# mfkiwl/coxgraph

Hardware: AMD Instinct MI355X
Metric: 640x480 depth frames/sec fused (TSDF, 5 cm voxels) per node; submap registrations/sec reported alongside (higher is better)
Workload: dtype f32; 1 GPU; configs[1]: 1 client per GPU, 640x480 synthetic depth stream, 5 cm voxels, merged integrator semantics (the reference's configured method is fast; bit-exact vs CPU oracle), points resident in HBM; points_per_frame=307200, method=merged, clients=1

## Files before the change

### coxgraph_amd/capi.py

```python
import ctypes as C
import os
import numpy as np

COX_OK = 0
STATUS = {
    0: "COX_OK", -1: "COX_ERR_INVALID_ARG", -2: "COX_ERR_NO_DEVICE", -3: "COX_ERR_OUT_OF_MEMORY",
    -4: "COX_ERR_POOL_EXHAUSTED", -5: "COX_ERR_INDEX_RANGE", -6: "COX_ERR_UNSUPPORTED",
    -7: "COX_ERR_BUFFER_TOO_SMALL", -8: "COX_ERR_INTERNAL", -9: "COX_ERR_COMM",
}
METHODS = {"simple": 0, "merged": 1, "fast": 2, "projective": 3}
QUERY_MODES = {"nearest": 0, "interpolate": 1, "adaptive": 2}
Q_VALUE, Q_TRILINEAR, Q_GRADIENT = 1, 2, 4
R_HIT, R_NORMAL, R_COLOR, R_BUDGET = 1, 2, 4, 8
VOXELS_PER_BLOCK = 4096


class CoxError(RuntimeError):
    def __init__(self, status, what):
        super().__init__(f"{what}: {STATUS.get(status, status)}")
        self.status = status


class TsdfConfig(C.Structure):
    _fields_ = [
# ... 49 lines not shown


def _ptr(t):
    if t is None:
        return None
    return C.c_void_p(t.data_ptr() if hasattr(t, "data_ptr") else int(t))


def _stream(s):
    return C.c_void_p(getattr(s, "cuda_stream", s) or 0)


def _pose(T):
    T = np.ascontiguousarray(T, np.float32)
    assert T.shape == (7,)
    return T


def _intrinsics(w, h, K):
    if K is None:
        from . import synth
        K = synth.INTRINSICS[(w, h)]
    K = np.ascontiguousarray(K, np.float32)
    assert K.shape == (4,)
    return K


def _config(eng, Struct, default_symbol, overrides):
    c = Struct()
    eng.fn(default_symbol, None)(C.byref(c))
    for k, v in overrides.items():
        if not hasattr(c, k):
            raise AttributeError(k)
        if isinstance(getattr(c, k), C.Array):
            v = type(getattr(c, k))(*np.asarray(v).ravel().tolist())
        setattr(c, k, v)
    return c


def _esdf_config(eng, max_distance_m=None, min_distance_m=None, default_distance_m=None, min_weight=None):
    if max_distance_m is not None and default_distance_m is None:
        default_distance_m = max_distance_m
    given = dict(max_distance_m=max_distance_m, min_distance_m=min_distance_m, default_distance_m=default_distance_m, min_weight=min_weight)
    return _config(eng, EsdfConfig, "esdf_config_default", {k: v for k, v in given.items() if v is not None})


class Engine:

    def __init__(self, lib_path, prefix):
        if not os.path.exists(lib_path):
            raise FileNotFoundError(lib_path)
        self.lib = C.CDLL(lib_path)
        self.prefix = prefix
        self.path = lib_path
        self._status_fns = {}

    def fn(self, name, restype=C.c_int):
        f = getattr(self.lib, self.prefix + name)
        f.restype = restype
        return f

    def has(self, name):
        return hasattr(self.lib, self.prefix + name)

    def check(self, status, what):
        if status != COX_OK:
            raise CoxError(status, what)

    def call(self, name, *args):
        try:
            f = self._status_fns[name]
        except KeyError:
            f = self._status_fns[name] = self.lib[self.prefix + name]
            f.restype = C.c_int
        status = f(*args)
        if status != COX_OK:
            raise CoxError(status, name)

    def default_config(self, **overrides):
        return _config(self, TsdfConfig, "tsdf_config_default", overrides)

    def device_count(self):
        return int(self.fn("device_count")()) if self.has("device_count") else 0


class _Handle:
    _destroy = None
    _hattr = "h"
    _borrows = ()
    eng = None
    h = None

    @classmethod
    def _adopt(cls, eng, handle, **attrs):
        self = cls.__new__(cls)
        self.eng = eng
        setattr(self, cls._hattr, handle)
        for k, v in attrs.items():
            setattr(self, k, v)
        return self

    def _guard(self, name):
        for a in self._borrows:
            if not getattr(self, a).h:
                raise CoxError(-1, name + " (the layer is closed)")
        return getattr(self, self._hattr)

    def _call(self, name, *args):
        self.eng.call(name, self._guard(name), *args)

    def _download(self, name, shapes, place=lambda arrays, cap: (*arrays, cap), query=None, also_ok=()):
        h, f, n = self._guard(name), self.eng.fn(name), C.c_uint64()
        status = f(h, *place([None] * len(shapes), C.c_uint64(0)), C.byref(n))
        if status not in also_ok:
            self.eng.check(status, query or name)
        out = tuple(np.zeros((int(n.value), *shape), dtype) for shape, dtype in shapes)
        if n.value:
            self.eng.check(f(h, *place([_fp(a) for a in out], C.c_uint64(n.value)), C.byref(n)), name)
        return out

    def close(self):
        h = getattr(self, self._hattr)
        if h:
            self.eng.fn(self._destroy, None)(h)
            setattr(self, self._hattr, C.c_void_p())

    def __del__(self):
        try:
            self.close()
        except Exception:
            pass


class Layer(_Handle):
    _destroy = "layer_destroy"

    def __init__(self, eng, voxel_size, voxels_per_side=16, device=0, capacity_blocks=0):
        self.eng = eng
        self.voxel_size = float(voxel_size)
        self.h = C.c_void_p()
        eng.call("layer_create", C.c_float(voxel_size), C.c_int(voxels_per_side), C.c_int(device), C.c_uint64(capacity_blocks), C.byref(self.h))

    def clear(self):
        self._call("layer_clear")

    def stats(self):
        n, b = C.c_uint64(), C.c_uint64()
        self._call("layer_stats", C.byref(n), C.byref(b))
        return int(n.value), int(b.value)

    def download(self):
        return self._download("layer_download", (((3,), np.int32), ((VOXELS_PER_BLOCK, 3), np.uint32)), query="layer_download(query)")

    def merge_from(self, other, T_B_A=None):
        self.eng.call("layer_merge", other.h, None if T_B_A is None else _fp(_pose(T_B_A)), self.h)

    def registration_points(self, min_voxel_weight=1.0, max_voxel_distance=0.3):
        return self._download("layer_registration_points", (((5,), np.float32),),
                              lambda a, cap: (C.c_float(min_voxel_weight), C.c_float(max_voxel_distance), *a, cap))[0]

    def surface_obb(self):
        mn, mx, n = np.zeros(3, np.float32), np.zeros(3, np.float32), C.c_uint64()
        self._call("layer_surface_obb", _fp(mn), _fp(mx), C.byref(n))
        return mn, mx, int(n.value)

    def esdf(self, max_distance_m=None, min_distance_m=None, default_distance_m=None, min_weight=None):
# ... 1342 lines not shown
```

### coxgraph_amd/csrc/cox_frontend.hpp

```cpp
#pragma once

constexpr u32 kDepthTile = 2048;
__device__ __forceinline__ bool depth_valid(float d) { return isfinite(d) && d > 0.0f; }
__global__ void __launch_bounds__(256) k_depth_count(const float* __restrict__ depth, u32 n, u32* __restrict__ tile_sums) {
  __shared__ u32 lds[4];
  const u32 n_tiles = (n + kDepthTile - 1) / kDepthTile;
  for (u32 tile = blockIdx.x; tile < n_tiles; tile += gridDim.x) {
    u32 c = 0;
#pragma unroll
    for (u32 q = 0; q < kDepthTile / 256; ++q) {
      const u32 i = tile * kDepthTile + q * 256 + threadIdx.x;
      c += (i < n && depth_valid(depth[i])) ? 1u : 0u;
    }
    u32 tot;
    (void)block_exclusive_scan<4>(c, &tot, lds);
    if (threadIdx.x == 0) tile_sums[tile] = tot;
  }
}
__global__ void __launch_bounds__(256) k_depth_points(const float* __restrict__ depth, const uint8_t* __restrict__ rgba, int w, int h, float fx, float fy,
                                                      float cx, float cy, const u32* __restrict__ tile_sums, float* __restrict__ xyz,
                                                      uint8_t* __restrict__ rgba_out, u32* __restrict__ n_out) {
  __shared__ u32 lds[4], lds2[4];
  const u32 n = static_cast<u32>(w) * static_cast<u32>(h);
  const u32 n_tiles = (n + kDepthTile - 1) / kDepthTile;
  for (u32 tile = blockIdx.x; tile < n_tiles; tile += gridDim.x) {
    u32 below = 0;
    for (u32 t = threadIdx.x; t < tile; t += 256) below += tile_sums[t];
    u32 base;
    (void)block_exclusive_scan<4>(below, &base, lds2);
    const u32 i0 = tile * kDepthTile + threadIdx.x * 8;
    float d[8];
    u32 c = 0;
#pragma unroll
    for (u32 q = 0; q < 8; ++q) {
      d[q] = (i0 + q < n) ? depth[i0 + q] : 0.0f;
      c += depth_valid(d[q]) ? 1u : 0u;
    }
    u32 tot;
    u32 o = base + block_exclusive_scan<4>(c, &tot, lds);
#pragma unroll
    for (u32 q = 0; q < 8; ++q) {
      if (!depth_valid(d[q])) continue;
      const u32 i = i0 + q;
      const u32 u = i % static_cast<u32>(w), v = i / static_cast<u32>(w);
      const float xn = (static_cast<float>(u) - cx) / fx;
      const float yn = (static_cast<float>(v) - cy) / fy;
      xyz[3 * o] = d[q] * xn;
      xyz[3 * o + 1] = d[q] * yn;
      xyz[3 * o + 2] = d[q];
      if (rgba_out) reinterpret_cast<u32*>(rgba_out)[o] = rgba ? reinterpret_cast<const u32*>(rgba)[i] : 0u;
      ++o;
    }
    if (tile + 1 == n_tiles && threadIdx.x == 0) *n_out = base + tot;
  }
}

typedef u32 U32x4 __attribute__((ext_vector_type(4)));
constexpr int kCopyGroups = 8;
struct HostSegment {
  U32x4* dst;
  const U32x4* src;
  size_t n16;
  u32 tail_words;
};
__device__ __forceinline__ void copy_segment_from_host(const HostSegment& g) {
  const size_t stride = static_cast<size_t>(gridDim.x) * blockDim.x;
  size_t i = blockIdx.x * static_cast<size_t>(blockDim.x) + threadIdx.x;
  for (; i + 3 * stride < g.n16; i += 4 * stride) {
    const U32x4 a = __builtin_nontemporal_load(&g.src[i]);
    const U32x4 b = __builtin_nontemporal_load(&g.src[i + stride]);
    const U32x4 c = __builtin_nontemporal_load(&g.src[i + 2 * stride]);
    const U32x4 d = __builtin_nontemporal_load(&g.src[i + 3 * stride]);
    g.dst[i] = a;
    g.dst[i + stride] = b;
    g.dst[i + 2 * stride] = c;
    g.dst[i + 3 * stride] = d;
  }
  for (; i < g.n16; i += stride) g.dst[i] = __builtin_nontemporal_load(&g.src[i]);
  if (blockIdx.x == 0 && threadIdx.x < g.tail_words)
    reinterpret_cast<u32*>(g.dst + g.n16)[threadIdx.x] = reinterpret_cast<const u32*>(g.src + g.n16)[threadIdx.x];
}
__global__ void __launch_bounds__(256) k_copy_from_host(const HostSegment a, const HostSegment b) {
  copy_segment_from_host(a);
  if (b.dst) copy_segment_from_host(b);
}

__global__ void __launch_bounds__(256) k_selftest_division(u64 n, u64 seed, u32* __restrict__ mismatches) {
  u64 bad = 0;
  for (u64 i = blockIdx.x * static_cast<u64>(blockDim.x) + threadIdx.x; i < n; i += static_cast<u64>(gridDim.x) * blockDim.x) {
    u64 z = seed + 0x9E3779B97F4A7C15ull * (i + 1);
    z = (z ^ (z >> 30)) * 0xBF58476D1CE4E5B9ull;
    z = (z ^ (z >> 27)) * 0x94D049BB133111EBull;
    z ^= z >> 31;
    const u32 a = static_cast<u32>(z), b = static_cast<u32>(z >> 32);
    float D, N;
    if ((i & 3) == 0) {
      D = static_cast<float>((b % 200000u) + 1u);
    } else {
      D = __uint_as_float(((b & 0x007FFFFFu) | (((b >> 23) % 80u + 87u) << 23)));
    }
    N = __uint_as_float((a & 0x807FFFFFu) | ((((a >> 23) & 0xFFu) % 80u + 87u) << 23));
    const float r0 = __builtin_amdgcn_rcpf(D);
    const float r = __builtin_fmaf(__builtin_fmaf(-D, r0, 1.0f), r0, r0);
    const float q0 = N * r;
    const float e0 = __builtin_fmaf(-D, q0, N);
    const float q1 = __builtin_fmaf(e0, r, q0);
    const float e1 = __builtin_fmaf(-D, q1, N);
    const float q = __builtin_fmaf(e1, r, q1);
    const float ref = N / D;
    if (__float_as_uint(q) != __float_as_uint(ref)) ++bad;
  }
  if (bad) atomicAdd(mismatches, static_cast<u32>(bad > 0xFFFFFFFFull ? 0xFFFFFFFFull : bad));
}

__global__ void __launch_bounds__(1024) k_scan_small(const u32* __restrict__ in, u32* __restrict__ out, const u32* __restrict__ d_n, u32 n_max,
                                                     u32* __restrict__ d_total) {
  __shared__ u32 lds[16];
  const u32 n = min(*d_n, n_max);
  u32 carry = 0;
  for (u32 base = 0; base < n; base += 1024 * 4) {
    const u32 i0 = base + threadIdx.x * 4;
    u32 v[4], sum = 0;
#pragma unroll
    for (int q = 0; q < 4; ++q) {
      v[q] = (i0 + q < n) ? in[i0 + q] : 0u;
      sum += v[q];
    }
    u32 total;
    u32 ex = carry + block_exclusive_scan<16>(sum, &total, lds);
#pragma unroll
    for (int q = 0; q < 4; ++q) {
      if (i0 + q < n) out[i0 + q] = ex;
      ex += v[q];
    }
    carry += total;
  }
  if (threadIdx.x == 0) *d_total = carry;
}

__global__ void __launch_bounds__(1024) k_scan_small2(const u32* __restrict__ in_a, u32* __restrict__ out_a, u32* __restrict__ total_a, const u32* __restrict__ in_b,
                                                      u32* __restrict__ out_b, u32* __restrict__ total_b, const u32* __restrict__ d_n, u32 n_max) {
  __shared__ u32 lds[16];
  const u32 n = min(*d_n, n_max);
  for (int which = 0; which < 2; ++which) {
    const u32* __restrict__ in = which ? in_b : in_a;
    u32* __restrict__ out = which ? out_b : out_a;
    u32 carry = 0;
    for (u32 base = 0; base < n; base += 1024 * 4) {
      const u32 i0 = base + threadIdx.x * 4;
      u32 v[4], sum = 0;
#pragma unroll
      for (int q = 0; q < 4; ++q) {
        v[q] = (i0 + q < n) ? in[i0 + q] : 0u;
        sum += v[q];
      }
      u32 total;
      u32 ex = carry + block_exclusive_scan<16>(sum, &total, lds);
#pragma unroll
      for (int q = 0; q < 4; ++q) {
        if (i0 + q < n) out[i0 + q] = ex;
        ex += v[q];
      }
      carry += total;
    }
    if (threadIdx.x == 0) *(which ? total_b : total_a) = carry;
  }
}
```

### coxgraph_amd/csrc/cox_integrator.hip

```cpp
#include <hip/hip_runtime.h>

#include <algorithm>
#include <chrono>
#include <cmath>
#include <cstring>
#include <limits>
#include <new>
#include <string>
#include <vector>

#include "../../include/coxgraph_hip_history.h"
#include "../../include/coxgraph_hip_selftest.h"
#include "cox_host.hpp"
#include "cox_plan.hpp"
#include "cox_sort.hpp"
#include "cox_threads.hpp"

using namespace cox;
using cox_plan::IntegratorPlan;
using cox_plan::LayerUpdate;

#include "cox_frame.hpp"
#include "cox_raygen.hpp"
#include "cox_walk.hpp"
#include "cox_pieces.hpp"
#include "cox_fast.hpp"
#include "cox_apply_records.hpp"
#include "cox_apply_tile.hpp"
#include "cox_frontend.hpp"

static_assert(cox_plan::kAxisCapSmall == kAxisCapSmall && cox_plan::kTileShift == kTileShift && cox_plan::kBigChunk == kBigChunk &&
                  cox_plan::kBigChunkMin == kBigChunkMin && cox_plan::kFastMaxRounds == kFastMaxRounds && cox_plan::kFastShortMax == kFastShortMax &&
                  cox_plan::kFastRelaxGroups == kFastRelaxGroups && cox_plan::kCopyGroups == kCopyGroups,
              "cox_plan.hpp decides with the kernels' own constants");

constexpr int kStatRing = 8;
constexpr int kFrameSets = 6;
constexpr int kStageSets = 3;
constexpr int kInputSets = kFrameSets;
using cox_plan::kNumStages;

struct FrameSet {
  FrameParams* d_params = nullptr;
  Counters* cnt = nullptr;
  RayArrays rays{};
  u64* fh_keys = nullptr;
  u32* fh_first = nullptr;
  hipEvent_t done = nullptr;
  hipEvent_t params_copied = nullptr;
  hipEvent_t hand[kNumStages - 1] = {};
  bool used = false;
};
struct BundleSet {
  u32 *pslot = nullptr, *skey[2] = {nullptr, nullptr}, *sval[2] = {nullptr, nullptr}, *bstart = nullptr;
  u32 *hrank = nullptr, *head = nullptr;
  SortInfo* sort_info = nullptr;
  hipEvent_t done = nullptr;
  bool used = false;
};
struct RecordSet {
  u32 *rec_key[2] = {nullptr, nullptr}, *rec_ray[2] = {nullptr, nullptr};
  u32 *piece_front = nullptr, *piece_back = nullptr, *piece_wsum = nullptr;
  uint8_t* lin8 = nullptr;
  u32 *pkey[2] = {nullptr, nullptr}, *pstart[2] = {nullptr, nullptr}, *prl[2] = {nullptr, nullptr};
  u64* pbkey = nullptr;
  u32 *plen = nullptr, *pdest = nullptr;
  u32* touched_slots = nullptr;
  u64* ft_keys = nullptr;
  u32* ft_ord = nullptr;
  int4* ord_info = nullptr;
  u32 *blk_beg = nullptr, *blk_end = nullptr;
  u32 *big_of_tile = nullptr, *big_acc = nullptr;
  u32* blk_list = nullptr;
  uint2* big_chunks = nullptr;
  u32 big_chunk_cap = 0;
  SortInfo* sort_info = nullptr;
  hipEvent_t done = nullptr;
  bool used = false;
};

using cox_plan::kFastCap0Max;
struct VisitSet {
  u32 *key[2] = {nullptr, nullptr}, *val[2] = {nullptr, nullptr};
  u64 *vhash = nullptr, *shash = nullptr;
  u32 *vray = nullptr, *pos_of = nullptr, *sinfo = nullptr, *voff = nullptr;
  u32 cap = 0;
  int sorted = 0;
  hipEvent_t done = nullptr;
  bool used = false;
};
struct FastState {
  u64 *fhash = nullptr, *table_start = nullptr, *table_obs = nullptr;
  u32 *fresh = nullptr, *rank = nullptr;
  u32* cap[kFrameSets] = {};
  u32* reach[kFrameSets] = {};
  VisitSet vs0[2];
  VisitSet vs1;
  u32* long_list = nullptr;
  u32* d_stats = nullptr;
  u64 off_start = 0, off_obs = 0;
  int reset_counter = 0;
  uint64_t frames = 0;
};

static std::mutex g_submitters_mutex;
// ... 1376 lines not shown
  COX_ENTRY();
  if (!I) return COX_ERR_INVALID_ARG;
  if (obs && !cox_internal_obs_matches(obs, I->layer)) return COX_ERR_INVALID_ARG;
  COX_HIP(hipSetDevice(I->layer->device));
  if (I->proj) return cox_proj_attach_history(I->proj, obs);
  COX_TRY(sync_all(I));
  if (obs && !I->ev_obs_read) {
    COX_TRY(make_event(I, &I->ev_obs_read));
    for (hipEvent_t& e : I->obs_read) COX_TRY(make_event(I, &e));
  }
  I->obs = obs;
  for (bool& u : I->obs_used) u = false;
  return COX_OK;
}

int cox_integrator_sync(cox_integrator_t* I) {
  COX_ENTRY();
  if (!I) return COX_ERR_INVALID_ARG;
  COX_HIP(hipSetDevice(I->layer->device));
  if (I->proj) return cox_proj_sync(I->proj);
  return integrator_finish(I);
}

int cox_integrator_last_stats(cox_integrator_t* I, cox_frame_stats* stats) {
  COX_ENTRY();
  if (!I || !stats) return COX_ERR_INVALID_ARG;
  COX_HIP(hipSetDevice(I->layer->device));
  if (I->proj) return cox_proj_last_stats(I->proj, stats);
  COX_TRY(sync_all(I));
  COX_TRY(fold_counters(I));
  *stats = I->last;
  return COX_OK;
}

int cox_integrator_set_profiling(cox_integrator_t* I, int on) {
  COX_ENTRY();
  if (!I) return COX_ERR_INVALID_ARG;
  I->profiling = on > 0;
  I->profile_every = on > 1 ? static_cast<u32>(on) : 1u;
  if (on > 0 && !I->proj && !I->timeline && !I->plan.timeline.empty()) {
    I->timeline = fopen(I->plan.timeline.c_str(), "a");
    if (I->timeline && hipEventCreate(&I->timeline_ref) == hipSuccess) {
      COX_HIP(hipSetDevice(I->layer->device));
      COX_TRY(sync_all(I));
      COX_HIP(hipEventRecord(I->timeline_ref, I->st[0]));
      fprintf(I->timeline, "# integrator %p method %d\n", static_cast<void*>(I), I->method);
    }
  }
  return COX_OK;
}

int cox_integrator_kernel_time(cox_integrator_t* I, double* apply_ms, uint64_t* apply_launches, int reset) {
  COX_ENTRY();
  if (!I) return COX_ERR_INVALID_ARG;
  if (I->proj) return COX_ERR_UNSUPPORTED;
  COX_HIP(hipSetDevice(I->layer->device));
  int st = integrator_finish(I);
  if (apply_ms) *apply_ms = I->class_ms[COX_KC_APPLY];
  if (apply_launches) *apply_launches = I->class_regions[COX_KC_APPLY];
  if (reset) {
    I->class_ms[COX_KC_APPLY] = 0.0;
    I->class_regions[COX_KC_APPLY] = 0;
  }
  return st;
}

int cox_selftest_division(int device, uint64_t n, uint64_t seed, uint64_t* mismatches) {
  COX_ENTRY();
  if (!mismatches) return COX_ERR_INVALID_ARG;
  int ndev = 0;
  if (hipGetDeviceCount(&ndev) != hipSuccess || device < 0 || device >= ndev) return COX_ERR_NO_DEVICE;
  COX_HIP(hipSetDevice(device));
  u32* d = nullptr;
  COX_HIP(hipMalloc(reinterpret_cast<void**>(&d), sizeof(u32)));
  COX_HIP(hipMemset(d, 0, sizeof(u32)));
  hipLaunchKernelGGL(k_selftest_division, dim3(4096), dim3(256), 0, nullptr, n, seed, d);
  u32 h = 0;
  COX_HIP(hipMemcpy(&h, d, sizeof(u32), hipMemcpyDeviceToHost));
  (void)hipFree(d);
  *mismatches = h;
  return COX_OK;
}

int cox_selftest_scan_small(int device, const uint32_t* in_a, const uint32_t* in_b, uint32_t len, uint32_t n_max, uint32_t d_n, uint32_t sentinel,
                            uint32_t* out1_a, uint32_t* out1_b, uint32_t* out2_a, uint32_t* out2_b, uint32_t totals[4]) {
  COX_ENTRY();
  int ndev = 0;
  if (hipGetDeviceCount(&ndev) != hipSuccess || device < 0 || device >= ndev) return COX_ERR_NO_DEVICE;
  if (!totals || len < std::min(d_n, n_max) || (len && (!in_a || !in_b || !out1_a || !out1_b || !out2_a || !out2_b))) return COX_ERR_INVALID_ARG;
  COX_HIP(hipSetDevice(device));
  const size_t words = std::max<size_t>(len, 1);
  u32* d = nullptr;
  COX_HIP(hipMalloc(reinterpret_cast<void**>(&d), (6 * words + 5) * sizeof(u32)));
  u32 *d_in[2] = {d, d + words}, *d_out = d + 2 * words, *d_cnt = d + 6 * words, *d_tot = d_cnt + 1;
  const int st = [&]() -> int {
    if (len) {
      COX_HIP(hipMemcpy(d_in[0], in_a, len * sizeof(u32), hipMemcpyHostToDevice));
      COX_HIP(hipMemcpy(d_in[1], in_b, len * sizeof(u32), hipMemcpyHostToDevice));
    }
    COX_HIP(hipMemsetD32(reinterpret_cast<hipDeviceptr_t>(d_out), static_cast<int>(sentinel), 4 * words));
    COX_HIP(hipMemsetD32(reinterpret_cast<hipDeviceptr_t>(d_tot), static_cast<int>(sentinel), 4));
    COX_HIP(hipMemcpy(d_cnt, &d_n, sizeof(u32), hipMemcpyHostToDevice));
    COX_HIP(hipDeviceSynchronize());
    hipLaunchKernelGGL(k_scan_small, dim3(1), dim3(1024), 0, nullptr, d_in[0], d_out, d_cnt, n_max, d_tot);
    hipLaunchKernelGGL(k_scan_small, dim3(1), dim3(1024), 0, nullptr, d_in[1], d_out + words, d_cnt, n_max, d_tot + 1);
    hipLaunchKernelGGL(k_scan_small2, dim3(1), dim3(1024), 0, nullptr, d_in[0], d_out + 2 * words, d_tot + 2, d_in[1], d_out + 3 * words, d_tot + 3, d_cnt, n_max);
    COX_HIP(hipGetLastError());
    COX_HIP(hipDeviceSynchronize());
    uint32_t* outs[4] = {out1_a, out1_b, out2_a, out2_b};
    for (int k = 0; k < 4 && len; ++k) COX_HIP(hipMemcpy(outs[k], d_out + k * words, len * sizeof(u32), hipMemcpyDeviceToHost));
    COX_HIP(hipMemcpy(totals, d_tot, 4 * sizeof(u32), hipMemcpyDeviceToHost));
    return COX_OK;
  }();
  (void)hipFree(d);
  return st;
}

constexpr u32 kSelftestGuard = 64;
static int selftest_guard_touched(const u32* d_guard, u32 sentinel, uint32_t* touched) {
  u32 g[kSelftestGuard];
  COX_HIP(hipMemcpy(g, d_guard, sizeof(g), hipMemcpyDeviceToHost));
  *touched = 0;
  for (u32 v : g) *touched += v != sentinel ? 1u : 0u;
  return COX_OK;
}

int cox_selftest_depth_points(int device, const float* depth, const uint8_t* rgba, int w, int h, const float K[4], uint32_t grid, int want_rgba,
                              uint32_t sentinel, float* xyz_out, uint8_t* rgba_out, uint32_t* tile_sums_out, uint32_t* n_out, uint32_t guard_touched[3]) {
  COX_ENTRY();
  int ndev = 0;
  if (hipGetDeviceCount(&ndev) != hipSuccess || device < 0 || device >= ndev) return COX_ERR_NO_DEVICE;
  if (!depth || !K || w <= 0 || h <= 0 || static_cast<uint64_t>(w) * h > (1ull << 24) || grid > 65535u || !xyz_out || !rgba_out || !tile_sums_out ||
      !n_out || !guard_touched)
    return COX_ERR_INVALID_ARG;
  COX_HIP(hipSetDevice(device));
  const size_t n = static_cast<size_t>(w) * h, tiles = depth_tiles(static_cast<u32>(n)), G = kSelftestGuard;
  const size_t o_rgba_in = n, o_xyz = 2 * n, o_rgba = o_xyz + 3 * n + G, o_tiles = o_rgba + n + G, o_n = o_tiles + tiles + G, words = o_n + 1;
  DevBuf<u32> buf;
  COX_TRY(buf.alloc(words));
  u32* d = buf.p;
  COX_HIP(hipMemcpy(d, depth, n * sizeof(float), hipMemcpyHostToDevice));
  if (rgba) COX_HIP(hipMemcpy(d + o_rgba_in, rgba, n * 4, hipMemcpyHostToDevice));
  COX_HIP(hipMemsetD32(reinterpret_cast<hipDeviceptr_t>(d + o_xyz), static_cast<int>(sentinel), words - o_xyz));
  COX_HIP(hipDeviceSynchronize());
  launch_depth_convert(reinterpret_cast<const float*>(d), rgba ? reinterpret_cast<const uint8_t*>(d + o_rgba_in) : nullptr, w, h, K, grid, d + o_tiles,
                       reinterpret_cast<float*>(d + o_xyz), want_rgba ? reinterpret_cast<uint8_t*>(d + o_rgba) : nullptr, d + o_n, nullptr);
  COX_HIP(hipGetLastError());
  COX_HIP(hipDeviceSynchronize());
  COX_HIP(hipMemcpy(xyz_out, d + o_xyz, 3 * n * sizeof(float), hipMemcpyDeviceToHost));
  COX_HIP(hipMemcpy(rgba_out, d + o_rgba, n * 4, hipMemcpyDeviceToHost));
  COX_HIP(hipMemcpy(tile_sums_out, d + o_tiles, tiles * sizeof(u32), hipMemcpyDeviceToHost));
  COX_HIP(hipMemcpy(n_out, d + o_n, sizeof(u32), hipMemcpyDeviceToHost));
  COX_TRY(selftest_guard_touched(d + o_xyz + 3 * n, sentinel, &guard_touched[0]));
  COX_TRY(selftest_guard_touched(d + o_rgba + n, sentinel, &guard_touched[1]));
  COX_TRY(selftest_guard_touched(d + o_tiles + tiles, sentinel, &guard_touched[2]));
  return COX_OK;
}

int cox_selftest_copy_from_host(int device, const uint32_t* a, uint64_t words_a, const uint32_t* b, uint64_t words_b, int groups, uint32_t sentinel,
                                uint32_t* out_a, uint32_t* out_b, uint32_t guard_touched[2]) {
  COX_ENTRY();
  int ndev = 0;
  if (hipGetDeviceCount(&ndev) != hipSuccess || device < 0 || device >= ndev) return COX_ERR_NO_DEVICE;
  constexpr uint64_t kMaxWords = 1ull << 24;
  if (groups < 1 || groups > 1024 || words_a > kMaxWords || words_b > kMaxWords || !guard_touched || (words_a && (!a || !out_a)) || (!b && words_b) ||
      (words_b && !out_b))
// ... 118 lines not shown
```

### coxgraph_amd/csrc/cox_raygen.hpp

```cpp
#pragma once

__global__ void __launch_bounds__(256) k_rays_simple(const FrameParams* __restrict__ Pp, RayArrays R,
                                                     Counters* cnt) {
  const FrameParams P = *Pp;
  const u32 seq = blockIdx.x * blockDim.x + threadIdx.x;
  if (seq == 0) cnt->n_ray_slots = P.n_points;
  if (seq >= P.n_points) return;
  const u32 idx = mixed_index(seq, P.n_points);
  const F3 p{P.xyz[3 * idx], P.xyz[3 * idx + 1], P.xyz[3 * idx + 2]};
  bool clearing = false;
  const bool valid = point_valid(P, p, &clearing);
  u32 nsteps = 0, flags = 0;
  if (valid) {
    const F3 pg = transform_point(P, p);
    Dda d;
    dda_setup(d, P, pg, clearing);
    if (d.range_error) atomicOr(&cnt->err, kErrRange);
    nsteps = d.nsteps;
    flags = 1u | (clearing ? 2u : 0u);
    R.px[seq] = pg.x;
    R.py[seq] = pg.y;
    R.pz[seq] = pg.z;
    R.w[seq] = voxel_weight(P, p);
    R.color[seq] = pack_rgba_wire(P.rgba, idx);
// ... 167 lines not shown
      if (c) atomicAdd(&totals[d], c);
    }
  }
}
struct BundleView {
  const u32* key[2];
  const u32* val[2];
  const SortInfo* info;
};
constexpr u32 kHeadLdsTiles = 2048;
struct BundleBounds {
  static constexpr bool kActive = true;
  static constexpr u32 kLdsWords = 2 * kHeadLdsTiles + 8;
  const FrameParams* Pp;
  const u32* tile_heads;
  const u32* hrank;
  const u32* pslot;
  u32* bstart;
  Counters* cnt;
  u64* fh_keys;
  u32* fh_first;
  u32 fh_mask;
  __device__ __forceinline__ void begin(u32 n, u32* lds) const {
    u32* scratch = lds + 2 * kHeadLdsTiles;
    const u32 n_tiles = (n + kHeadTile - 1) / kHeadTile;
    u32 carry = 0;
    for (u32 cls = 0; cls < 2; ++cls) {
      for (u32 b = 0; b < n_tiles; b += 256) {
        const u32 t = b + threadIdx.x;
        const u32 v = (t < n_tiles) ? tile_heads[4 * t + cls] : 0u;
        u32 tot;
        const u32 ex = block_exclusive_scan<4>(v, &tot, scratch);
        if (t < n_tiles && t < kHeadLdsTiles) lds[cls * kHeadLdsTiles + t] = carry + ex;
        carry += tot;
      }
    }
    if (blockIdx.x == 0) {
      u32 v = 0;
      for (u32 t = threadIdx.x; t < n_tiles; t += 256) v += tile_heads[4 * t + 2];
      u32 n_valid;
      (void)block_exclusive_scan<4>(v, &n_valid, scratch);
      if (threadIdx.x == 0) {
        cnt->n_rays = carry;
        cnt->n_ray_slots = carry;
        cnt->n_sorted_valid = n_valid;
      }
    }
    if (threadIdx.x == 0) {
      scratch[4] = n;
      scratch[5] = Pp->np2;
    }
    __syncthreads();
  }
  struct Fetched {
    u32 ord, slot;
  };
  __device__ __forceinline__ bool wants(u32 key, u32 val, const u32* lds) const {
    const u32 np2 = lds[2 * kHeadLdsTiles + 5];
    return key != kInvalid && (key & (np2 - 1u)) == val;
  }
  __device__ __forceinline__ Fetched fetch(u32 key, u32 val, const u32* lds) const {
    const u32 n = lds[2 * kHeadLdsTiles + 4], np2 = lds[2 * kHeadLdsTiles + 5];
    const u32 cls = key >= np2 ? 1u : 0u;
    const u32 tile = val >> kHeadTileShift;
    u32 ord;
    if (tile < kHeadLdsTiles) {
      ord = lds[cls * kHeadLdsTiles + tile];
    } else {
      ord = lds[cls * kHeadLdsTiles + kHeadLdsTiles - 1];
      for (u32 t = kHeadLdsTiles - 1; t < tile; ++t) ord += tile_heads[4 * t + cls];
    }
    ord += hrank[val];
    return Fetched{ord < n ? ord : kInvalid, fh_keys ? pslot[mixed_index(val, n)] : kInvalid};
  }
  __device__ __forceinline__ void commit(const Fetched& f, u32 pos) const {
    if (f.ord != kInvalid) bstart[f.ord] = pos;
    if (f.slot <= fh_mask) {
      fh_keys[f.slot] = kEmptyKey;
      fh_first[f.slot] = 0xFFFFFFFFu;
    }
  }
};

typedef float MergeOp __attribute__((ext_vector_type(4)));

__device__ __forceinline__ u32 piece_bound(const Dda& d, u32 axis_cap) {
  const u32 ns = d.nsteps;
  if (ns == 0) return 0;
  const u32 gen = ns + 1;
  const u32 g0 = min(d.n_axis[0] + 2, gen), g1 = min(d.n_axis[1] + 2, gen), g2 = min(d.n_axis[2] + 2, gen);
  if (d.sgn[0] == 0 || d.sgn[1] == 0 || d.sgn[2] == 0 || g0 > axis_cap || g1 > axis_cap || g2 > axis_cap || ns > 3 * axis_cap) return ns;
  const u32 b = (ns + 63) / 64 + (d.n_axis[2] + 1) + ((d.n_axis[0] + 1) / 16 + 1) + ((d.n_axis[1] + 1) / 16 + 1) + 4;
  return min(b, ns);
}

template <u32 kAxisCap>
__device__ void wave_touch_ray(const FrameParams& P, const RayArrays& R, const FrameBlocks& B, u32 r, u32 ns, u32 flags, Dda d, u64 own_key, float* tl, u32* path,
                               u32 lane, u32* __restrict__ park, Counters* cnt, const u64* __restrict__ fh_keys, u32 fh_mask);

struct MergeWalk {
  FrameBlocks blocks;
  u32* path;
  u32 path_stride;
  u32 rec_cap;
  const u64* fh_keys;
  u32 fh_mask;
};

template <bool kWalk>
__global__ void __launch_bounds__(256) k_bundle_merge(const FrameParams* __restrict__ Pp, BundleView V, const u32* __restrict__ bstart, RayArrays R, Counters* cnt,
                                                      u32 piece_axis_cap, MergeWalk walk) {
  const FrameParams P = *Pp;
  const u32 np2 = P.np2;
  const float* __restrict__ xyz = P.xyz;
  const uint8_t* __restrict__ rgba = P.rgba;
  typedef const float __attribute__((address_space(1))) * GlobalF32;
  typedef const u32 __attribute__((address_space(1))) * GlobalU32;
  const GlobalF32 gxyz = (GlobalF32)xyz;
  const GlobalU32 grgba = (GlobalU32)rgba;
  const u32 spar = uniform_u32(V.info->parity & 1u);
  const u32* __restrict__ skey = V.key[spar];
  const u32* __restrict__ sval = V.val[spar];
  __shared__ MergeOp ops[4][64][4];
  const u32 n_bundles = uniform_u32(cnt->n_rays);
  const u32 n_valid = uniform_u32(cnt->n_sorted_valid);
  const u32 tid = blockIdx.x * blockDim.x + threadIdx.x;
  const u32 nthreads = gridDim.x * blockDim.x;
  const u32 lane = lane_id();
  const u32 role = lane & 3u;
  MergeOp(*tbl)[4] = ops[threadIdx.x >> 6];
  for (u32 task = uniform_u32(tid >> 6); task < 2 * n_bundles; task += nthreads >> 6) {
    const u32 m = task >> 1;
    const bool colour_wave = (task & 1u) != 0;
    const u32 begin = uniform_u32(bstart[m]);
    const u32 next_start = uniform_u32(bstart[min(m + 1u, n_bundles - 1u)]);
    const u32 end = (m + 1 < n_bundles) ? next_start : n_valid;
    if (colour_wave && rgba == nullptr) {
      if (lane == 0) {
        R.color[m] = 0u;
        reinterpret_cast<u32*>(R.q)[static_cast<size_t>(m) * 8u + 5u] = 0u;
      }
      continue;
    }
    auto gather = [&](bool has, u32 sv, float& x, float& y, float& z, u32& c) {
      x = 0.0f;
      y = 0.0f;
      z = 0.0f;
      c = 0u;
      if (has) {
        const u32 idx = mixed_index(sv, P.n_points);
        x = gxyz[3 * idx];
        y = gxyz[3 * idx + 1];
        z = gxyz[3 * idx + 2];
        if (colour_wave) c = grgba[idx];
      }
    };
    const u32 key0 = skey[begin];
    const u32 sv_a = (begin + lane < end) ? sval[begin + lane] : 0u;
    u32 sv_b = (begin + 64u + lane < end) ? sval[begin + 64u + lane] : 0u;
    float npx, npy, npz;
    u32 ncol;
    gather(begin + lane < end, sv_a, npx, npy, npz, ncol);
    const bool clearing = uniform_u32(key0) >= np2;
    if (!colour_wave && lane == 0) atomicMax(&cnt->shard[m & 63u][kShMaxBundle], end - begin);
    float val = 0.0f;
    float W = 0.0f;
    u64 key = 0;
    bool done = false;
    for (u32 base = begin; base < end && !done; base += 64) {
      const u32 i = base + lane;
      const u32 cnt_in = min(64u, end - base);
      const float px = npx, py = npy, pz = npz;
      const u32 col = rgba_wire_order(ncol);
      const float w = (i < end) ? voxel_weight(P, F3{px, py, pz}) : 0.0f;
      gather(i + 64u < end, sv_b, npx, npy, npz, ncol);
      sv_b = (i + 128u < end) ? sval[i + 128u] : 0u;
      if (base == begin && !colour_wave) {
        const F3 pg = transform_point(P, F3{readlane_f32(px, 0), readlane_f32(py, 0), readlane_f32(pz, 0)});
        key = pack_key(grid_index(pg.x * P.voxel_size_inv), grid_index(pg.y * P.voxel_size_inv), grid_index(pg.z * P.voxel_size_inv));
      }
      bool used = (lane < cnt_in) && !(w < kEps);
      if (clearing) {
        const u64 um = __ballot(used);
        used = used && (lane == static_cast<u32>(__ffsll(static_cast<long long>(um))) - 1u);
        if (um) done = true;
      }
      float Wpre;
      const u64 in_mask = (cnt_in == 64) ? ~0ull : ((1ull << cnt_in) - 1ull);
      if (!clearing && (__ballot(w == 1.0f) & in_mask) == in_mask && W == truncf(W) && W < 8388608.0f) {
        Wpre = W + static_cast<float>(lane);
      } else {
        float run = W;
        Wpre = W;
        const u64 used_mask = __ballot(used);
        for (u32 k = 0; k < cnt_in; ++k) {
          if (lane == k) Wpre = run;
          const float wk = readlane_f32(w, k);
          if ((used_mask >> k) & 1ull) run += wk;
        }
      }
      const float den = Wpre + w;
      const float Wnext = used ? den : Wpre;
      const bool d_ok = !used || (den >= 9.094947e-13f && den <= 1.0995116e12f);
      {
        MergeOp* row = tbl[lane];
        const MergeOp ident{1.0f, 0.0f, 1.0f, 1.0f};
        if (!used) {
#pragma unroll
          for (u32 c = 0; c < 4; ++c) row[c] = ident;
        } else if (!colour_wave) {
          const float r0 = __builtin_amdgcn_rcpf(den);
          const float r = __builtin_fmaf(__builtin_fmaf(-den, r0, 1.0f), r0, r0);
          row[0] = MergeOp{Wpre, px * w, den, r};
          row[1] = MergeOp{Wpre, py * w, den, r};
          row[2] = MergeOp{Wpre, pz * w, den, r};
          row[3] = ident;
        } else {
          const float fa = Wpre / den, fb = w / den;
#pragma unroll
          for (u32 c = 0; c < 4; ++c) row[c] = MergeOp{fa, static_cast<float>(static_cast<int>((col >> (8u * c)) & 255u)) * fb, 1.0f, 0.0f};
        }
      }
      wave_lds_handover();
      MergeOp nxt = tbl[0][role];
      if (!colour_wave) {
        const float val_in = val;
        float n_lo = 1.0f, n_hi = 1.0f;
        MergeOp a0 = tbl[0][role], a1 = tbl[1][role], a2 = tbl[2][role], a3 = tbl[3][role];
#define COX_MERGE_STEP(op)                                  \
  {                                                         \
    const float N = val * (op).x + (op).y;                  \
    n_lo = fminf(n_lo, fabsf(N));                           \
    n_hi = fmaxf(n_hi, fabsf(N));                           \
    const float q0 = N * (op).w;                            \
    const float e0 = __builtin_fmaf(-(op).z, q0, N);        \
    const float q1 = __builtin_fmaf(e0, (op).w, q0);        \
    const float e1 = __builtin_fmaf(-(op).z, q1, N);        \
    val = __builtin_fmaf(e1, (op).w, q1);                   \
  }
        for (u32 k = 0; k < cnt_in; k += 8) {
          const u32 kb = (k + 4) & 63u;
          const MergeOp b0 = tbl[kb][role], b1 = tbl[kb + 1][role], b2 = tbl[kb + 2][role], b3 = tbl[kb + 3][role];
          __builtin_amdgcn_sched_barrier(0);
          COX_MERGE_STEP(a0)
          COX_MERGE_STEP(a1)
          COX_MERGE_STEP(a2)
          COX_MERGE_STEP(a3)
          __builtin_amdgcn_sched_barrier(0);
          const u32 ka = (k + 8) & 63u;
          a0 = tbl[ka][role];
          a1 = tbl[ka + 1][role];
          a2 = tbl[ka + 2][role];
          a3 = tbl[ka + 3][role];
          __builtin_amdgcn_sched_barrier(0);
          COX_MERGE_STEP(b0)
          COX_MERGE_STEP(b1)
          COX_MERGE_STEP(b2)
          COX_MERGE_STEP(b3)
          __builtin_amdgcn_sched_barrier(0);
        }
#undef COX_MERGE_STEP
        const bool bad = (lane < 3) && !(n_lo >= 9.094947e-13f && n_hi <= 1.0995116e12f);
        if (__ballot(bad || !d_ok)) {
          val = val_in;
          nxt = tbl[0][role];
          for (u32 k = 0; k < cnt_in; ++k) {
            const MergeOp op = nxt;
            nxt = tbl[(k + 1) & 63u][role];
            val = (val * op.x + op.y) / op.z;
          }
        }
      } else {
#define COX_COLOUR_STEP(op)                                 \
  {                                                         \
    const float x = val * (op).x + (op).y;                  \
    const float t = truncf(x);                              \
    val = (x - t >= 0.5f) ? t + 1.0f : t;                   \
  }
        MergeOp a0 = tbl[0][role], a1 = tbl[1][role], a2 = tbl[2][role], a3 = tbl[3][role];
        for (u32 k = 0; k < cnt_in; k += 8) {
          const u32 kb = (k + 4) & 63u;
          const MergeOp b0 = tbl[kb][role], b1 = tbl[kb + 1][role], b2 = tbl[kb + 2][role], b3 = tbl[kb + 3][role];
          __builtin_amdgcn_sched_barrier(0);
          COX_COLOUR_STEP(a0)
          COX_COLOUR_STEP(a1)
          COX_COLOUR_STEP(a2)
          COX_COLOUR_STEP(a3)
          __builtin_amdgcn_sched_barrier(0);
          const u32 ka = (k + 8) & 63u;
          a0 = tbl[ka][role];
          a1 = tbl[ka + 1][role];
          a2 = tbl[ka + 2][role];
          a3 = tbl[ka + 3][role];
          __builtin_amdgcn_sched_barrier(0);
          COX_COLOUR_STEP(b0)
          COX_COLOUR_STEP(b1)
          COX_COLOUR_STEP(b2)
          COX_COLOUR_STEP(b3)
          __builtin_amdgcn_sched_barrier(0);
        }
#undef COX_COLOUR_STEP
      }
      wave_lds_handover();
      W = readlane_f32(Wnext, cnt_in - 1);
    }
    if (colour_wave) {
      u32 mcolor = 0;
#pragma unroll
      for (u32 c = 0; c < 4; ++c) mcolor |= (static_cast<u32>(static_cast<int>(readlane_f32(val, c))) & 255u) << (8u * c);
      if (lane == 0) {
        R.color[m] = mcolor;
        reinterpret_cast<u32*>(R.q)[static_cast<size_t>(m) * 8u + 5u] = mcolor;
      }
    } else {
      const float mx = readlane_f32(val, 0), my = readlane_f32(val, 1), mz = readlane_f32(val, 2);
      auto write_ray = [&](const F3& pg, const Dda& d, u32 flags) {
        if (d.range_error) atomicOr(&cnt->err, kErrRange);
        R.px[m] = pg.x;
        R.py[m] = pg.y;
        R.pz[m] = pg.z;
        R.w[m] = W;
        R.flags[m] = flags;
        R.key[m] = key;
        R.nsteps[m] = d.nsteps;
        if (piece_axis_cap) R.pbound[m] = piece_bound(d, piece_axis_cap);
        {
          const F3 dv = pg - F3{P.tx, P.ty, P.tz};
          typedef float F4 __attribute__((ext_vector_type(4)));
          F4* q = reinterpret_cast<F4*>(R.q + static_cast<size_t>(m) * 8u);
          q[0] = F4{dv.x, dv.y, dv.z, sqrtf(dot3(dv, dv))};
          R.q[static_cast<size_t>(m) * 8u + 4u] = W;
        }
      };
      if constexpr (kWalk) {
        static_assert(6 * kAxisCapSmall * sizeof(u32) <= sizeof(ops[0]), "the walk's scratch fits the wave's operand table");
        const F3 pg = transform_point(P, F3{mx, my, mz});
        Dda d;
        dda_setup(d, P, pg, clearing);
        const u32 ns = d.nsteps;
        const bool fits = ns <= walk.path_stride && (static_cast<u64>(m) + 1ull) * walk.path_stride <= static_cast<u64>(walk.rec_cap);
        const u32 flags = 1u | (clearing ? 2u : 0u) | (fits ? 0u : kRayNoPath);
        if (lane == 0) write_ray(pg, d, flags);
        if (ns != 0) {
          float* tl = reinterpret_cast<float*>(tbl);
          wave_touch_ray<kAxisCapSmall>(P, R, walk.blocks, m, ns, flags, d, key, tl, reinterpret_cast<u32*>(tl + 3 * kAxisCapSmall), lane,
                                        fits ? walk.path + m * walk.path_stride : nullptr, cnt, walk.fh_keys, walk.fh_mask);
          wave_lds_handover();
        }
      } else if (lane == 0) {
        const F3 pg = transform_point(P, F3{mx, my, mz});
        Dda d;
        dda_setup(d, P, pg, clearing);
        write_ray(pg, d, 1u | (clearing ? 2u : 0u));
      }
    }
  }
}
```

### include/coxgraph_hip_selftest.h

```cpp
#ifndef COXGRAPH_HIP_SELFTEST_H_
#define COXGRAPH_HIP_SELFTEST_H_
#include "coxgraph_hip.h"
#include "coxgraph_hip_depthfuse.h"
#include "coxgraph_hip_stereo_filter.h"

#ifdef __cplusplus
extern "C" {
#endif

typedef struct cox_selftest_sort_args {
  int32_t rb;
  uint32_t n_max;
  int32_t use_d_n;
  uint32_t d_n;
  uint32_t n_hint;
  int32_t bits_on_device;
  uint32_t nbits;
  uint32_t base;
  int32_t max_passes;
  int32_t pass0_counted;
  int32_t hook;
  int32_t repeat;
  const uint32_t* repeat_nbits;
  uint32_t sentinel;
  uint32_t pad0;
  const uint32_t* keys;
  const uint32_t* vals;
  const uint32_t* extra;
  const uint32_t* aux;
  uint32_t* k0;
  uint32_t* v0;
  uint32_t* x0;
  uint32_t* k1;
  uint32_t* v1;
  uint32_t* x1;
  uint32_t* hook_pos;
  uint32_t* hook_aux;
  uint32_t* hook_count;
  int32_t result_buffer;
  uint32_t totals_nonzero;
  uint32_t guard_touched;
  uint32_t pad1;
} cox_selftest_sort_args;

int cox_selftest_sort(int device, cox_selftest_sort_args* args);

int cox_selftest_scan(int device, const uint32_t* in, uint32_t n_max, int use_d_n, uint32_t d_n, uint32_t n_hint, int in_place,
                      int want_total, uint32_t sentinel, uint32_t* out, uint32_t* total);

int cox_selftest_scan_small(int device, const uint32_t* in_a, const uint32_t* in_b, uint32_t len, uint32_t n_max, uint32_t d_n,
                            uint32_t sentinel, uint32_t* out1_a, uint32_t* out1_b, uint32_t* out2_a, uint32_t* out2_b,
                            uint32_t totals[4]);

int cox_selftest_depth_points(int device, const float* depth, const uint8_t* rgba, int w, int h, const float K[4], uint32_t grid, int want_rgba,
                              uint32_t sentinel, float* xyz_out, uint8_t* rgba_out, uint32_t* tile_sums_out, uint32_t* n_out,
                              uint32_t guard_touched[3]);

int cox_selftest_copy_from_host(int device, const uint32_t* a, uint64_t words_a, const uint32_t* b, uint64_t words_b, int groups, uint32_t sentinel,
                                uint32_t* out_a, uint32_t* out_b, uint32_t guard_touched[2]);

int cox_selftest_depthfuse_box(float voxel_size, const cox_depthfuse_config* cfg, const float T_G_C[7], int w, int height, const float K[4],
                               int32_t lo[3], uint32_t dims[3]);

int cox_selftest_stereo_filters(int device, const uint16_t* disparity, int w, int h, const cox_stereo_filter_config* cfg, uint16_t* median_out,
                                uint32_t* labels_out, uint16_t* filtered_out, uint64_t counts[4], uint32_t guard_touched[3]);

#ifdef __cplusplus
}
#endif
#endif
```

Before: 8762 frames/s.

## Shorten serial merge-step division chain with deferred exactness check

The per-voxel merge chain used two Newton corrections per step to get a correctly rounded quotient. Each step now applies one correction, so the serial dependency is N→q0→e0→q1. The second correction is computed off the critical path, one step late, and any bit it would change is accumulated in `q_moved`; if any step moved, the existing ballot fallback replays the chain exactly. The row reciprocal now comes from `1.0f/D`, and the colour rounding step becomes a branch-free truncation difference. A GPU selftest and Python binding check the one-correction quotient against IEEE division for several operand classes; the risk is extra register pressure and more fallback replays when rounding ties are common.

Result: no change. 8723 frames/s, median of 2 (-0.4%).

```diff
diff --git a/coxgraph_amd/capi.py b/coxgraph_amd/capi.py
--- a/coxgraph_amd/capi.py
+++ b/coxgraph_amd/capi.py
@@ -155,6 +155,11 @@
 
     def device_count(self):
         return int(self.fn("device_count")()) if self.has("device_count") else 0
+
+    def selftest_merge_chain(self, n, seed, operand_class, device=0):
+        out = (C.c_uint64 * 3)()
+        self.call("selftest_merge_chain", C.c_int(device), C.c_uint64(n), C.c_uint64(seed), C.c_int(operand_class), out)
+        return tuple(int(v) for v in out)
 
 
 class _Handle:
diff --git a/coxgraph_amd/csrc/cox_frontend.hpp b/coxgraph_amd/csrc/cox_frontend.hpp
--- a/coxgraph_amd/csrc/cox_frontend.hpp
+++ b/coxgraph_amd/csrc/cox_frontend.hpp
@@ -85,32 +85,80 @@
   if (b.dst) copy_segment_from_host(b);
 }
 
+__device__ __forceinline__ u64 selftest_mix(u64 seed, u64 i) {
+  u64 z = seed + 0x9E3779B97F4A7C15ull * (i + 1);
+  z = (z ^ (z >> 30)) * 0xBF58476D1CE4E5B9ull;
+  z = (z ^ (z >> 27)) * 0x94D049BB133111EBull;
+  return z ^ (z >> 31);
+}
+__device__ __forceinline__ float selftest_in_range(u32 bits, bool with_sign) {
+  return __uint_as_float((bits & (with_sign ? 0x807FFFFFu : 0x007FFFFFu)) | ((((bits >> 23) & 0xFFu) % 80u + 87u) << 23));
+}
+
+struct SelftestStep {
+  float val, M, A, D;
+};
+__device__ __forceinline__ SelftestStep selftest_operands(int cls, u64 seed, u64 i) {
+  const u64 z = selftest_mix(seed, i);
+  const u32 a = static_cast<u32>(z), b = static_cast<u32>(z >> 32);
+  switch (cls) {
+    case 1: {
+      const float W = static_cast<float>(b & 0x007FFFFFu);
+      const u64 y = selftest_mix(seed ^ 0xA5A5A5A5ull, i);
+      const float val = (static_cast<float>(static_cast<u32>(y) >> 8) * (1.0f / 16777216.0f) - 0.5f) * 20.0f;
+      const float p = (static_cast<float>(static_cast<u32>(y >> 32) >> 8) * (1.0f / 16777216.0f) - 0.5f) * 20.0f;
+      return SelftestStep{val, W, p, W + 1.0f};
+    }
+    case 2: {
+      const float D = __uint_as_float((b & 0x007FFFFFu) | (((b >> 23) % 40u + 107u) << 23));
+      const float m = __uint_as_float((a & 0x807FFFFFu) | ((((a >> 23) & 0xFFu) % 40u + 107u) << 23));
+      const double half_ulp = static_cast<double>(__uint_as_float(__float_as_uint(fabsf(m)) & 0x7F800000u)) * (1.0 / 16777216.0);
+      const double tie = static_cast<double>(m) + (m < 0.0f ? -half_ulp : half_ulp);
+      return SelftestStep{static_cast<float>(static_cast<double>(D) * tie), 1.0f, 0.0f, D};
+    }
+    case 3: {
+      const u32 expo = ((b >> 23) % 80u + 87u) << 23;
+      return SelftestStep{selftest_in_range(a, true), 1.0f, 0.0f, __uint_as_float(expo | ((i & 1) ? 0x007FFFFFu : 0u))};
+    }
+    case 4: {
+      const u32 ed = 87u + ((b >> 23) & 1u) + ((b >> 24) & 1u) * 78u, en = 87u + ((a >> 23) & 1u) + ((a >> 24) & 1u) * 78u;
+      return SelftestStep{__uint_as_float((a & 0x807FFFFFu) | (en << 23)), 1.0f, 0.0f, __uint_as_float((b & 0x007FFFFFu) | (ed << 23))};
+    }
+    default: {
+      const float D = (i & 3) == 0 ? static_cast<float>((b % 200000u) + 1u)
+                                   : __uint_as_float((b & 0x007FFFFFu) | (((b >> 23) % 80u + 87u) << 23));
+      return SelftestStep{selftest_in_range(a, true), 1.0f, 0.0f, D};
+    }
+  }
+}
+
 __global__ void __launch_bounds__(256) k_selftest_division(u64 n, u64 seed, u32* __restrict__ mismatches) {
   u64 bad = 0;
   for (u64 i = blockIdx.x * static_cast<u64>(blockDim.x) + threadIdx.x; i < n; i += static_cast<u64>(gridDim.x) * blockDim.x) {
-    u64 z = seed + 0x9E3779B97F4A7C15ull * (i + 1);
-    z = (z ^ (z >> 30)) * 0xBF58476D1CE4E5B9ull;
-    z = (z ^ (z >> 27)) * 0x94D049BB133111EBull;
-    z ^= z >> 31;
-    const u32 a = static_cast<u32>(z), b = static_cast<u32>(z >> 32);
-    float D, N;
-    if ((i & 3) == 0) {
-      D = static_cast<float>((b % 200000u) + 1u);
-    } else {
-      D = __uint_as_float(((b & 0x007FFFFFu) | (((b >> 23) % 80u + 87u) << 23)));
-    }
-    N = __uint_as_float((a & 0x807FFFFFu) | ((((a >> 23) & 0xFFu) % 80u + 87u) << 23));
-    const float r0 = __builtin_amdgcn_rcpf(D);
-    const float r = __builtin_fmaf(__builtin_fmaf(-D, r0, 1.0f), r0, r0);
-    const float q0 = N * r;
-    const float e0 = __builtin_fmaf(-D, q0, N);
-    const float q1 = __builtin_fmaf(e0, r, q0);
-    const float e1 = __builtin_fmaf(-D, q1, N);
-    const float q = __builtin_fmaf(e1, r, q1);
-    const float ref = N / D;
+    const SelftestStep s = selftest_operands(0, seed, i);
+    MergeChainSide side;
+    const float q = merge_step(s.val, merge_row(s.M, s.A, s.D), side);
+    const float ref = (s.val * s.M + s.A) / s.D;
     if (__float_as_uint(q) != __float_as_uint(ref)) ++bad;
   }
   if (bad) atomicAdd(mismatches, static_cast<u32>(bad > 0xFFFFFFFFull ? 0xFFFFFFFFull : bad));
+}
+
+__global__ void __launch_bounds__(256) k_selftest_merge_chain(u64 n, u64 seed, int cls, unsigned long long* __restrict__ out) {
+  u32 bad1 = 0, bad2 = 0, moved = 0;
+  for (u64 i = blockIdx.x * static_cast<u64>(blockDim.x) + threadIdx.x; i < n; i += static_cast<u64>(gridDim.x) * blockDim.x) {
+    const SelftestStep s = selftest_operands(cls, seed, i);
+    MergeChainSide side;
+    const float q = merge_step(s.val, merge_row(s.M, s.A, s.D), side);
+    (void)side.finish(q);
+    const u32 q1 = __float_as_uint(q), q2 = q1 ^ side.q_moved, ref = __float_as_uint((s.val * s.M + s.A) / s.D);
+    bad1 += q1 != ref;
+    bad2 += q2 != ref;
+    moved += q1 != q2;
+  }
+  if (bad1) atomicAdd(&out[0], static_cast<unsigned long long>(bad1));
+  if (bad2) atomicAdd(&out[1], static_cast<unsigned long long>(bad2));
+  if (moved) atomicAdd(&out[2], static_cast<unsigned long long>(moved));
 }
 
 __global__ void __launch_bounds__(1024) k_scan_small(const u32* __restrict__ in, u32* __restrict__ out, const u32* __restrict__ d_n, u32 n_max,
diff --git a/coxgraph_amd/csrc/cox_integrator.hip b/coxgraph_amd/csrc/cox_integrator.hip
--- a/coxgraph_amd/csrc/cox_integrator.hip
+++ b/coxgraph_amd/csrc/cox_integrator.hip
@@ -21,6 +21,7 @@
 using cox_plan::LayerUpdate;
 
 #include "cox_frame.hpp"
+#include "cox_merge_step.hpp"
 #include "cox_raygen.hpp"
 #include "cox_walk.hpp"
 #include "cox_pieces.hpp"
@@ -1563,6 +1564,27 @@
   return COX_OK;
 }
 
+int cox_selftest_merge_chain(int device, uint64_t n, uint64_t seed, int operand_class, uint64_t out[3]) {
+  COX_ENTRY();
+  int ndev = 0;
+  if (hipGetDeviceCount(&ndev) != hipSuccess || device < 0 || device >= ndev) return COX_ERR_NO_DEVICE;
+  if (!out || operand_class < 0 || operand_class > 4 || n >= (1ull << 40)) return COX_ERR_INVALID_ARG;
+  COX_HIP(hipSetDevice(device));
+  unsigned long long* d = nullptr;
+  COX_HIP(hipMalloc(reinterpret_cast<void**>(&d), 3 * sizeof(unsigned long long)));
+  const int st = [&]() -> int {
+    COX_HIP(hipMemset(d, 0, 3 * sizeof(unsigned long long)));
+    hipLaunchKernelGGL(k_selftest_merge_chain, dim3(4096), dim3(256), 0, nullptr, n, seed, operand_class, d);
+    COX_HIP(hipGetLastError());
+    unsigned long long h[3] = {0, 0, 0};
+    COX_HIP(hipMemcpy(h, d, sizeof(h), hipMemcpyDeviceToHost));
+    for (int k = 0; k < 3; ++k) out[k] = h[k];
+    return COX_OK;
+  }();
+  (void)hipFree(d);
+  return st;
+}
+
 int cox_selftest_scan_small(int device, const uint32_t* in_a, const uint32_t* in_b, uint32_t len, uint32_t n_max, uint32_t d_n, uint32_t sentinel,
                             uint32_t* out1_a, uint32_t* out1_b, uint32_t* out2_a, uint32_t* out2_b, uint32_t totals[4]) {
   COX_ENTRY();
diff --git a/coxgraph_amd/csrc/cox_merge_step.hpp b/coxgraph_amd/csrc/cox_merge_step.hpp
--- /dev/null
+++ b/coxgraph_amd/csrc/cox_merge_step.hpp
@@ -0,0 +1,53 @@
+#pragma once
+
+typedef float MergeOp __attribute__((ext_vector_type(4)));
+
+__device__ __forceinline__ MergeOp merge_row(float M, float A, float D) { return MergeOp{M, A, D, 1.0f / D}; }
+__device__ __forceinline__ MergeOp merge_row_identity() { return MergeOp{1.0f, 0.0f, 1.0f, 1.0f}; }
+
+
+struct MergeChainSide {
+  float n_lo = 1.0f, n_hi = 1.0f;
+  u32 q_moved = 0u;
+  float pe = 0.0f, pr = 0.0f;
+  __device__ __forceinline__ bool finish(float q1) {
+    const float q2 = __builtin_fmaf(pe, pr, q1);
+    q_moved |= __float_as_uint(q2) ^ __float_as_uint(q1);
+    return q_moved != 0u || !(n_lo >= 9.094947e-13f && n_hi <= 1.0995116e12f);
+  }
+};
+
+__device__ __forceinline__ float merge_step(float val, const MergeOp& op, MergeChainSide& side) {
+  asm volatile("" : "+v"(side.q_moved));
+  const float N = val * op.x + op.y;
+  __builtin_amdgcn_sched_barrier(0);
+  const float q2 = __builtin_fmaf(side.pe, side.pr, val);
+  const float q0 = N * op.w;
+  __builtin_amdgcn_sched_barrier(0);
+  const float e0 = __builtin_fmaf(-op.z, q0, N);
+  side.q_moved |= __float_as_uint(q2) ^ __float_as_uint(val);
+  __builtin_amdgcn_sched_barrier(0);
+  const float q1 = __builtin_fmaf(e0, op.w, q0);
+  side.n_lo = fminf(side.n_lo, fabsf(N));
+  side.n_hi = fmaxf(side.n_hi, fabsf(N));
+  __builtin_amdgcn_sched_barrier(0);
+  side.pe = __builtin_fmaf(-op.z, q1, N);
+  side.pr = op.w;
+  return q1;
+}
+
+__device__ __forceinline__ void merge_group_end(float& val, MergeChainSide& s) {
+  float r;
+  asm volatile("v_mov_b32 %0, %1" : "=&v"(r) : "v"(s.pr));
+  s.pr = r;
+  asm volatile("" : "+v"(val), "+v"(s.n_lo), "+v"(s.n_hi), "+v"(s.q_moved), "+v"(s.pe), "+v"(s.pr));
+}
+
+__device__ __forceinline__ MergeOp colour_row(float fa, float cb) { return MergeOp{fa, cb, 2.0f * fa, 2.0f * cb}; }
+__device__ __forceinline__ MergeOp colour_row_identity() { return MergeOp{1.0f, 0.0f, 2.0f, 0.0f}; }
+
+__device__ __forceinline__ float colour_step(float val, const MergeOp& op) {
+  const float x = val * op.x + op.y;
+  const float x2 = val * op.z + op.w;
+  return truncf(x2) - truncf(x);
+}
diff --git a/coxgraph_amd/csrc/cox_raygen.hpp b/coxgraph_amd/csrc/cox_raygen.hpp
--- a/coxgraph_amd/csrc/cox_raygen.hpp
+++ b/coxgraph_amd/csrc/cox_raygen.hpp
@@ -273,7 +273,6 @@
   }
 };
 
-typedef float MergeOp __attribute__((ext_vector_type(4)));
 
 __device__ __forceinline__ u32 piece_bound(const Dda& d, u32 axis_cap) {
   const u32 ns = d.nsteps;
@@ -395,40 +394,28 @@
       const bool d_ok = !used || (den >= 9.094947e-13f && den <= 1.0995116e12f);
       {
         MergeOp* row = tbl[lane];
-        const MergeOp ident{1.0f, 0.0f, 1.0f, 1.0f};
         if (!used) {
+          const MergeOp ident = colour_wave ? colour_row_identity() : merge_row_identity();
 #pragma unroll
           for (u32 c = 0; c < 4; ++c) row[c] = ident;
         } else if (!colour_wave) {
-          const float r0 = __builtin_amdgcn_rcpf(den);
-          const float r = __builtin_fmaf(__builtin_fmaf(-den, r0, 1.0f), r0, r0);
-          row[0] = MergeOp{Wpre, px * w, den, r};
-          row[1] = MergeOp{Wpre, py * w, den, r};
-          row[2] = MergeOp{Wpre, pz * w, den, r};
-          row[3] = ident;
+          row[0] = merge_row(Wpre, px * w, den);
+          row[1] = merge_row(Wpre, py * w, den);
+          row[2] = merge_row(Wpre, pz * w, den);
+          row[3] = merge_row_identity();
         } else {
           const float fa = Wpre / den, fb = w / den;
 #pragma unroll
-          for (u32 c = 0; c < 4; ++c) row[c] = MergeOp{fa, static_cast<float>(static_cast<int>((col >> (8u * c)) & 255u)) * fb, 1.0f, 0.0f};
+          for (u32 c = 0; c < 4; ++c) row[c] = colour_row(fa, static_cast<float>(static_cast<int>((col >> (8u * c)) & 255u)) * fb);
         }
       }
       wave_lds_handover();
       MergeOp nxt = tbl[0][role];
       if (!colour_wave) {
         const float val_in = val;
-        float n_lo = 1.0f, n_hi = 1.0f;
+        MergeChainSide side;
         MergeOp a0 = tbl[0][role], a1 = tbl[1][role], a2 = tbl[2][role], a3 = tbl[3][role];
-#define COX_MERGE_STEP(op)                                  \
-  {                                                         \
-    const float N = val * (op).x + (op).y;                  \
-    n_lo = fminf(n_lo, fabsf(N));                           \
-    n_hi = fmaxf(n_hi, fabsf(N));                           \
-    const float q0 = N * (op).w;                            \
-    const float e0 = __builtin_fmaf(-(op).z, q0, N);        \
-    const float q1 = __builtin_fmaf(e0, (op).w, q0);        \
-    const float e1 = __builtin_fmaf(-(op).z, q1, N);        \
-    val = __builtin_fmaf(e1, (op).w, q1);                   \
-  }
+#define COX_MERGE_STEP(op) val = merge_step(val, op, side);
         for (u32 k = 0; k < cnt_in; k += 8) {
           const u32 kb = (k + 4) & 63u;
           const MergeOp b0 = tbl[kb][role], b1 = tbl[kb + 1][role], b2 = tbl[kb + 2][role], b3 = tbl[kb + 3][role];
@@ -437,6 +424,7 @@
           COX_MERGE_STEP(a1)
           COX_MERGE_STEP(a2)
           COX_MERGE_STEP(a3)
+          merge_group_end(val, side);
           __builtin_amdgcn_sched_barrier(0);
           const u32 ka = (k + 8) & 63u;
           a0 = tbl[ka][role];
@@ -448,10 +436,11 @@
           COX_MERGE_STEP(b1)
           COX_MERGE_STEP(b2)
           COX_MERGE_STEP(b3)
+          merge_group_end(val, side);
           __builtin_amdgcn_sched_barrier(0);
         }
 #undef COX_MERGE_STEP
-        const bool bad = (lane < 3) && !(n_lo >= 9.094947e-13f && n_hi <= 1.0995116e12f);
+        const bool bad = side.finish(val) && (lane < 3);
         if (__ballot(bad || !d_ok)) {
           val = val_in;
           nxt = tbl[0][role];
@@ -462,12 +451,7 @@
           }
         }
       } else {
-#define COX_COLOUR_STEP(op)                                 \
-  {                                                         \
-    const float x = val * (op).x + (op).y;                  \
-    const float t = truncf(x);                              \
-    val = (x - t >= 0.5f) ? t + 1.0f : t;                   \
-  }
+#define COX_COLOUR_STEP(op) val = colour_step(val, op);
         MergeOp a0 = tbl[0][role], a1 = tbl[1][role], a2 = tbl[2][role], a3 = tbl[3][role];
         for (u32 k = 0; k < cnt_in; k += 8) {
           const u32 kb = (k + 4) & 63u;
diff --git a/include/coxgraph_hip_selftest.h b/include/coxgraph_hip_selftest.h
--- a/include/coxgraph_hip_selftest.h
+++ b/include/coxgraph_hip_selftest.h
@@ -65,6 +65,8 @@
 int cox_selftest_stereo_filters(int device, const uint16_t* disparity, int w, int h, const cox_stereo_filter_config* cfg, uint16_t* median_out,
                                 uint32_t* labels_out, uint16_t* filtered_out, uint64_t counts[4], uint32_t guard_touched[3]);
 
+int cox_selftest_merge_chain(int device, uint64_t n, uint64_t seed, int operand_class, uint64_t out[3]);
+
 #ifdef __cplusplus
 }
 #endif
```
